# pola-rs/polars

Hardware: NVIDIA H100
Metric: group_by_agg_rows_per_sec (higher is better)
Workload: dtype int64/float64

## Files before the change

polars_b200/csrc/groupby_radix.cu:

```cuda
#include <algorithm>
#include <cstdlib>

#include "common.cuh"
#include "dev_utils.cuh"
#include "groupby.h"
#include "groupby_dev.cuh"

namespace plb {

constexpr int GBR_THREADS = 512;
constexpr int GBR_MAX_LOGB = 13;
constexpr int GBR_NCW = 31, GBR_NCT = GBR_NCW * 32;
constexpr unsigned GBR_NO_ROOM = 0xFFFFFFFFu;

struct GbRadixDev {
    uint64_t* recs;
    const unsigned long long* off;
    unsigned* cursor;
    unsigned* counts;
    int logB, roww;
    uint64_t* special;
    unsigned cap;
    int* status;
};

template <int KEY_ELEM> __device__ __forceinline__ void gbr_load_pair(const void* col, int64_t r0, int64_t n, uint64_t& a, uint64_t& b) {
    a = 0; b = 0;
    if (r0 + 1 < n) gb_load_pair<KEY_ELEM>(col, r0, a, b);
    else if (r0 < n) a = KEY_ELEM == 8 ? reinterpret_cast<const uint64_t*>(col)[r0] : reinterpret_cast<const uint32_t*>(col)[r0];
}
__device__ __forceinline__ void gbr_load_pair_rt(const void* col, int elem, int64_t r0, int64_t n, uint64_t& a, uint64_t& b) {
    if (elem == 8) gbr_load_pair<8>(col, r0, n, a, b); else gbr_load_pair<4>(col, r0, n, a, b);
}

template <int KEY_ELEM, int KEY_CANON>
__global__ void __launch_bounds__(512) k_gbr_hist(const void* __restrict__ keys, int64_t n, int logB, unsigned* __restrict__ counts) {
    extern __shared__ unsigned h_s[];
    const int B = 1 << logB;
    for (int i = threadIdx.x; i < B; i += blockDim.x) h_s[i] = 0;
    __syncthreads();
    const int64_t npairs = (n + 1) >> 1;
    for (int64_t p = (int64_t)blockIdx.x * blockDim.x + threadIdx.x; p < npairs; p += (int64_t)gridDim.x * blockDim.x) {
        uint64_t k0, k1;
        gbr_load_pair<KEY_ELEM>(keys, 2 * p, n, k0, k1);
        k0 = canon_key<KEY_CANON>(k0); k1 = canon_key<KEY_CANON>(k1);
        if (k0 != GB_EMPTY) atomicAdd(&h_s[(unsigned)(table_hash(k0) >> (64 - logB))], 1u);
        if (2 * p + 1 < n && k1 != GB_EMPTY) atomicAdd(&h_s[(unsigned)(table_hash(k1) >> (64 - logB))], 1u);
    }
    __syncthreads();
    for (int i = threadIdx.x; i < B; i += blockDim.x) if (h_s[i]) atomicAdd(&counts[i], h_s[i]);
}
__host__ __device__ __forceinline__ unsigned long long gbr_stream_records(unsigned long long rows, unsigned long long pad_units, unsigned pad_each, unsigned align) {
    rows += (rows < pad_units ? rows : pad_units) * pad_each;
    return (rows + align - 1) & ~(unsigned long long)(align - 1);
}
__global__ void __launch_bounds__(1024) k_gbr_offsets(const __grid_constant__ GbLayout L, const unsigned* __restrict__ counts, unsigned long long rows, int B, unsigned long long pad_units,
                                                      unsigned pad_each, unsigned align, unsigned long long* __restrict__ off, unsigned* __restrict__ cursor, uint64_t* __restrict__ special, int* __restrict__ status) {
// ... 17 lines not shown
            wsum[lane] = t - s;
        }
        __syncthreads();
        const unsigned long long incl = carry_s + wsum[warp] + x;
        if (i < B) off[i] = incl - c;
        __syncthreads();
        if (threadIdx.x == 1023) carry_s = incl;
        __syncthreads();
    }
    if (threadIdx.x == 0) off[B] = carry_s;
}

__device__ __forceinline__ void gbr_apply_special(const GbLayout& L, const GbBatch& Bt, uint64_t* sp, const uint64_t* raw) {
    atomicAdd(reinterpret_cast<unsigned long long*>(sp), 1ull);
    for (int c = 0; c < L.n_cols; c++)
        for (int k = L.col_kbegin[c]; k < L.col_kbegin[c + 1]; k++) {
            uint64_t* a = sp + 1 + L.wslot[k];
            const int dt = Bt.cols[c].dtype;
            switch (L.wop[k]) {
                case W_ADD_INT: atomicAdd(reinterpret_cast<unsigned long long*>(a), (unsigned long long)raw_to_int(dt, raw[c])); break;
                case W_ADD_F64: atomicAdd(reinterpret_cast<double*>(a), raw_to_f64(dt, raw[c])); break;
                case W_MIN_S64: atomicMin(reinterpret_cast<long long*>(a), (long long)raw_to_int(dt, raw[c])); break;
                case W_MAX_S64: atomicMax(reinterpret_cast<long long*>(a), (long long)raw_to_int(dt, raw[c])); break;
                case W_MIN_U64: atomicMin(reinterpret_cast<unsigned long long*>(a), (unsigned long long)raw[c]); break;
                case W_MAX_U64: atomicMax(reinterpret_cast<unsigned long long*>(a), (unsigned long long)raw[c]); break;
                case W_MIN_F64: { const double f = raw_to_f64(dt, raw[c]); if (f == f) atomicMin(reinterpret_cast<unsigned long long*>(a), (unsigned long long)f64_to_ordered(f)); break; }
                case W_MAX_F64: { const double f = raw_to_f64(dt, raw[c]); if (f == f) atomicMax(reinterpret_cast<unsigned long long*>(a), (unsigned long long)f64_to_ordered(f)); break; }
                default: break;
            }
        }
}

constexpr int GBR_RPT = 4;
template <int ROWW, int KEY_ELEM, int KEY_CANON, bool BULK>
__global__ void __launch_bounds__(GBR_THREADS) k_gbr_scatter(const __grid_constant__ GbLayout L, const __grid_constant__ GbBatch Bt, const __grid_constant__ GbRadixDev R) {
    constexpr int RPT = GBR_RPT, T = GBR_THREADS * RPT, THREADS = GBR_THREADS, NC = ROWW - 1;
    const int logB = R.logB, B = 1 << logB;
    extern __shared__ __align__(16) uint64_t gbr_smem[];
    uint64_t* stage = gbr_smem;
    unsigned* hist = reinterpret_cast<unsigned*>(stage + (size_t)(T + (BULK ? B : 0)) * ROWW);
    unsigned* start = hist + B;
    unsigned* gpos = start + B;
    uint16_t* sp = reinterpret_cast<uint16_t*>(gpos + B);
    __shared__ unsigned warp_tot[THREADS / 32];
    const int tid = threadIdx.x, lane = tid & 31, warp = tid >> 5;
    const int64_t n = Bt.n;
    const int64_t ntiles = (n + T - 1) / T;
    for (int64_t tile = blockIdx.x; tile < ntiles; tile += gridDim.x) {
        const int64_t base = tile * T;
        for (int p = tid; p < B; p += THREADS) hist[p] = 0;
        __syncthreads();
        uint64_t k[RPT]; unsigned pk[RPT];
#pragma unroll
        for (int j = 0; j < RPT / 2; j++) gbr_load_pair<KEY_ELEM>(Bt.keys, base + 2 * (int64_t)(j * THREADS + tid), n, k[2 * j], k[2 * j + 1]);
#pragma unroll
        for (int j = 0; j < RPT; j++) {
            const int64_t r = base + 2 * (int64_t)((j >> 1) * THREADS + tid) + (j & 1);
            pk[j] = 0xFFFFFFFFu;
            if (r < n) {
                k[j] = canon_key<KEY_CANON>(k[j]);
                if (k[j] == GB_EMPTY) pk[j] = 0xFFFFFFFEu;
                else { const unsigned b = (unsigned)(table_hash(k[j]) >> (64 - logB)); pk[j] = (b << 16) | atomicAdd(&hist[b], 1u); }
            }
        }
        __syncthreads();
        const int bins = (B + THREADS - 1) / THREADS;
        unsigned mine = 0;
        for (int q = 0; q < bins; q++) { const int p = tid * bins + q; if (p < B) { unsigned c = hist[p]; if (BULK) c = (c + 1u) & ~1u; mine += c; } }
        unsigned x = mine;
        for (int o = 1; o < 32; o <<= 1) { const unsigned y = __shfl_up_sync(0xffffffffu, x, o); if (lane >= o) x += y; }
        if (lane == 31) warp_tot[warp] = x;
        __syncthreads();
        if (warp == 0) {
            unsigned w = lane < THREADS / 32 ? warp_tot[lane] : 0, s = w;
            for (int o = 1; o < 32; o <<= 1) { const unsigned y = __shfl_up_sync(0xffffffffu, s, o); if (lane >= o) s += y; }
            if (lane < THREADS / 32) warp_tot[lane] = s - w;
        }
        __syncthreads();
        unsigned run = warp_tot[warp] + x - mine;
        for (int q = 0; q < bins; q++) {
            const int p = tid * bins + q;
            if (p < B) {
                const unsigned c = hist[p], cp = BULK ? ((c + 1u) & ~1u) : c;
                start[p] = run;
                unsigned g = cp ? atomicAdd(&R.cursor[p], cp) : 0u;
                if (g + cp > R.cap) { *R.status = 2; g = GBR_NO_ROOM; }
                gpos[p] = g;
                run += cp;
            }
        }
        if (BULK) bulk_wait_read0();
        __syncthreads();
        if (BULK) for (int p = tid; p < B; p += THREADS) { const unsigned c = hist[p]; if (c & 1u) { uint64_t* pad = stage + (size_t)(start[p] + c) * ROWW; pad[0] = GB_EMPTY;
#pragma unroll
                                                                                                      for (int w = 1; w < ROWW; w++) pad[w] = 0; } }
#pragma unroll
        for (int j = 0; j < RPT / 2; j++) {
            const int64_t r0 = base + 2 * (int64_t)(j * THREADS + tid);
            uint64_t v[NC > 0 ? NC : 1][2];
#pragma unroll
            for (int c = 0; c < NC; c++) gbr_load_pair_rt(Bt.cols[c].values, Bt.cols[c].elem, r0, n, v[c][0], v[c][1]);
#pragma unroll
            for (int e = 0; e < 2; e++) {
                const unsigned q = pk[2 * j + e];
                if (q == 0xFFFFFFFFu) continue;
                if (q == 0xFFFFFFFEu) {
                    uint64_t raw[NC > 0 ? NC : 1];
#pragma unroll
                    for (int c = 0; c < NC; c++) raw[c] = v[c][e];
                    gbr_apply_special(L, Bt, R.special, raw);
                    continue;
                }
                const unsigned bkt = q >> 16, pos = start[bkt] + (q & 0xFFFFu);
                uint64_t* rec = stage + (size_t)pos * ROWW;
                rec[0] = k[2 * j + e];
#pragma unroll
                for (int c = 0; c < NC; c++) rec[1 + c] = v[c][e];
                if (!BULK) sp[pos] = (uint16_t)bkt;
            }
        }
        if (BULK) fence_async_smem();
        __syncthreads();
        if (BULK) {
            for (int p = tid; p < B; p += THREADS) {
                const unsigned c = hist[p], cp = (c + 1u) & ~1u;
                if (cp && gpos[p] != GBR_NO_ROOM) bulk_s2g(R.recs + (R.off[p] + gpos[p]) * ROWW, stage + (size_t)start[p] * ROWW, cp * ROWW * 8);
            }
            bulk_commit();
        } else {
            const unsigned total = start[B - 1] + hist[B - 1];
            for (unsigned w = tid; w < total * ROWW; w += THREADS) {
                const unsigned row = w / ROWW, c = w - row * ROWW;
                const unsigned p = sp[row], g = gpos[p];
                if (g != GBR_NO_ROOM) R.recs[(R.off[p] + g + (row - start[p])) * ROWW + c] = stage[w];
            }
            __syncthreads();
        }
    }
    if (BULK) bulk_wait0();
}

constexpr int GBR_WC_THREADS = 256, GBR_WC_F = 4;
template <int ROWW> constexpr int gbr_wc_rpt() { return ROWW <= 3 ? 8 : 4; }
template <int ROWW, int KEY_ELEM, int RPT>
__device__ __forceinline__ void gbr_wc_load(const GbBatch& Bt, int64_t base, uint64_t (&k)[RPT], uint64_t (&v)[ROWW > 1 ? ROWW - 1 : 1][RPT]) {
#pragma unroll
    for (int j = 0; j < RPT / 2; j++) {
        const int64_t r0 = base + 2 * (int64_t)(j * GBR_WC_THREADS + threadIdx.x);
        gbr_load_pair<KEY_ELEM>(Bt.keys, r0, Bt.n, k[2 * j], k[2 * j + 1]);
#pragma unroll
        for (int c = 0; c < ROWW - 1; c++) gbr_load_pair_rt(Bt.cols[c].values, Bt.cols[c].elem, r0, Bt.n, v[c][2 * j], v[c][2 * j + 1]);
    }
}

template <int ROWW, int KEY_ELEM, int KEY_CANON>
__global__ void __launch_bounds__(GBR_WC_THREADS, 2) k_gbr_scatter_wc(const __grid_constant__ GbLayout L, const __grid_constant__ GbBatch Bt, const __grid_constant__ GbRadixDev R) {
    constexpr int THREADS = GBR_WC_THREADS, F = GBR_WC_F, RPT = gbr_wc_rpt<ROWW>(), T = THREADS * RPT, NC = ROWW - 1, NCX = NC > 0 ? NC : 1, CH = F * ROWW;
    constexpr unsigned NONE = 0xFFFFFFFFu;
    const int logB = R.logB, B = 1 << logB, tid = threadIdx.x;
    extern __shared__ __align__(16) uint64_t gbr_smem[];
    uint64_t* buf = gbr_smem;
    unsigned* fill = reinterpret_cast<unsigned*>(buf + (size_t)B * CH);
    const int64_t n = Bt.n, ntiles = (n + T - 1) / T;
    for (int p = tid; p < B; p += THREADS) fill[p] = 0;
    uint64_t k[RPT], v[NCX][RPT], kn[RPT], vn[NCX][RPT];
    if ((int64_t)blockIdx.x < ntiles) gbr_wc_load<ROWW, KEY_ELEM, RPT>(Bt, (int64_t)blockIdx.x * T, kn, vn);
    for (int64_t tile = blockIdx.x; tile < ntiles; tile += gridDim.x) {
#pragma unroll
        for (int e = 0; e < RPT; e++) { k[e] = kn[e];
#pragma unroll
                                        for (int c = 0; c < NC; c++) v[c][e] = vn[c][e]; }
        if (tile + gridDim.x < ntiles) gbr_wc_load<ROWW, KEY_ELEM, RPT>(Bt, (tile + gridDim.x) * T, kn, vn);
        const int64_t base = tile * T;
        unsigned pk[RPT];
#pragma unroll
        for (int e = 0; e < RPT; e++) {
            const int64_t r = base + 2 * (int64_t)((e >> 1) * THREADS + tid) + (e & 1);
            pk[e] = NONE;
            if (r < n) {
                k[e] = canon_key<KEY_CANON>(k[e]);
                if (k[e] == GB_EMPTY) {
                    uint64_t raw[NCX];
#pragma unroll
                    for (int c = 0; c < NC; c++) raw[c] = v[c][e];
                    gbr_apply_special(L, Bt, R.special, raw);
                } else pk[e] = (unsigned)(table_hash(k[e]) >> (64 - logB)) << 16;
            }
        }
        __syncthreads();
        unsigned last = 0;
#pragma unroll
        for (int e = 0; e < RPT; e++)
            if (pk[e] != NONE) { const unsigned s = atomicAdd(&fill[pk[e] >> 16], 1u); pk[e] |= s; last = max(last, s / F); }
        bulk_wait_read0();
        __syncthreads();
        for (unsigned r = 0;; r++) {
#pragma unroll
            for (int e = 0; e < RPT; e++) {
                const unsigned s = pk[e] & 0xFFFFu;
                if (pk[e] == NONE || s / F != r) continue;
                uint64_t* rec = buf + (size_t)(pk[e] >> 16) * CH + (s % F) * ROWW;
                rec[0] = k[e];
#pragma unroll
                for (int c = 0; c < NC; c++) rec[1 + c] = v[c][e];
            }
            fence_async_smem();
            const bool more = __syncthreads_or(last > r);
            const unsigned full = (r + 1) * F;
            for (int p0 = 0; p0 < B; p0 += 4 * THREADS) {
                unsigned g[4];
#pragma unroll
                for (int q = 0; q < 4; q++) {
                    const int p = p0 + q * THREADS + tid;
                    g[q] = NONE;
                    if (p < B) {
                        const unsigned f = fill[p];
                        if (f >= full) g[q] = atomicAdd(&R.cursor[p], (unsigned)F);
                        if (!more) fill[p] = f % F;
                    }
                }
#pragma unroll
                for (int q = 0; q < 4; q++) {
                    const int p = p0 + q * THREADS + tid;
                    if (g[q] == NONE) continue;
                    if (g[q] + F <= R.cap) bulk_s2g(R.recs + (R.off[p] + g[q]) * ROWW, buf + (size_t)p * CH, CH * 8);
                    else *R.status = 2;
                }
            }
            bulk_commit();
            if (!more) break;
            bulk_wait_read0();
            __syncthreads();
        }
    }
    __syncthreads();
    for (int p = tid; p < B; p += THREADS) {
        const unsigned f = fill[p];
        if (f == 0) continue;
        for (unsigned i = f; i < F; i++) buf[(size_t)p * CH + i * ROWW] = GB_EMPTY;
        fence_async_smem();
        const unsigned g = atomicAdd(&R.cursor[p], (unsigned)F);
        if (g + F <= R.cap) bulk_s2g(R.recs + (R.off[p] + g) * ROWW, buf + (size_t)p * CH, CH * 8);
        else *R.status = 2;
    }
    bulk_commit();
    bulk_wait0();
}

struct GbDenseDev { uint64_t* keys; uint32_t* first; uint32_t* len; uint64_t* words; int64_t Gb; unsigned long long* cursor; };

constexpr int GBR_NST = 2;
template <int ROWW>
__global__ void __launch_bounds__(1024) k_gbr_agg(const __grid_constant__ GbLayout L, const __grid_constant__ GbBatch Bt, const __grid_constant__ GbRadixDev R, const __grid_constant__ GbDenseDev D, unsigned S) {
    constexpr int NST = GBR_NST, CR = GBR_NCT, NC = ROWW - 1;
    extern __shared__ __align__(128) uint64_t gbr_smem2[];
    uint64_t* ring = gbr_smem2;
    uint64_t* tkey = ring + (size_t)NST * CR * ROWW;
    uint64_t* tacc = tkey + S;
    unsigned* tlen = reinterpret_cast<unsigned*>(tacc + (size_t)L.n_words * S);
    __shared__ uint64_t full[NST], empty[NST];
    __shared__ unsigned s_used, s_base;
    const int tid = threadIdx.x, warp = tid >> 5, lane = tid & 31, B = 1 << R.logB;
    if (*R.status == 2) return;
    if (tid == 0) { for (int s = 0; s < NST; s++) { mbar_init(&full[s], 1); mbar_init(&empty[s], GBR_NCW); } mbar_fence_init(); }
    __syncthreads();
    if (warp == GBR_NCW) {
        if (lane == 0) {
            unsigned q = 0;
            for (int p = blockIdx.x; p < B; p += gridDim.x) {
                const int64_t rows = (int64_t)R.cursor[p];
                const uint64_t* src = R.recs + R.off[p] * ROWW;
                const int nch = (int)((rows + CR - 1) / CR);
                for (int c = 0; c < nch; c++, q++) {
                    const int st = q % NST; const unsigned use = q / NST;
                    if (use > 0) while (!mbar_try_wait(&empty[st], (use - 1) & 1u)) {}
                    const int64_t crow = min((int64_t)CR, rows - (int64_t)c * CR);
                    const unsigned bytes = (unsigned)(((crow + 1) & ~(int64_t)1) * ROWW * 8);
                    mbar_expect_tx(&full[st], bytes);
                    bulk_g2s(ring + (size_t)st * CR * ROWW, src + (size_t)c * CR * ROWW, bytes, &full[st]);
                }
            }
        }
        return;
    }
    const unsigned max_used = S - (S >> 2);
    unsigned q = 0;
    for (int p = blockIdx.x; p < B; p += gridDim.x) {
        for (unsigned i = tid; i < S; i += GBR_NCT) { tkey[i] = GB_EMPTY; tlen[i] = 0; for (int w = 0; w < L.n_words; w++) tacc[(size_t)w * S + i] = L.init[w]; }
        if (tid == 0) s_used = 0;
        named_bar_sync(1, GBR_NCT);
        const int64_t rows = (int64_t)R.cursor[p];
        const int nch = (int)((rows + CR - 1) / CR);
        for (int c = 0; c < nch; c++, q++) {
            const int st = q % NST; const unsigned par = (q / NST) & 1u;
            while (!mbar_try_wait(&full[st], par)) {}
            const uint64_t* buf = ring + (size_t)st * CR * ROWW;
            const int crow = (int)min((int64_t)CR, rows - (int64_t)c * CR);
            uint64_t rec[ROWW];
            rec[0] = GB_EMPTY;
            if (tid < crow) {
#pragma unroll
                for (int w = 0; w < ROWW; w++) rec[w] = buf[tid * ROWW + w];
            }
            fence_async_smem();
            __syncwarp();
            if (lane == 0) mbar_arrive(&empty[st]);
            const uint64_t key = rec[0];
            if (key == GB_EMPTY) continue;
            unsigned slot = __umulhi((unsigned)((table_hash(key) << R.logB) >> 32), S);
            bool found = false;
            for (unsigned probes = 0; probes < 128u; probes++) {
                const uint64_t cur = *reinterpret_cast<volatile uint64_t*>(tkey + slot);
                if (cur == key) { found = true; break; }
                if (cur == GB_EMPTY) {
                    if (*reinterpret_cast<volatile unsigned*>(&s_used) >= max_used) break;
                    const unsigned long long old = atomicCAS(reinterpret_cast<unsigned long long*>(tkey + slot), (unsigned long long)GB_EMPTY, (unsigned long long)key);
                    if (old == GB_EMPTY) { atomicAdd(&s_used, 1u); found = true; break; }
                    if (old == key) { found = true; break; }
                }
                if (++slot == S) slot = 0;
            }
            if (!found) { *R.status = 1; continue; }
            if (L.need_len) atomicAdd(tlen + slot, 1u);
#pragma unroll
            for (int cix = 0; cix < NC; cix++) {
                const int dt = Bt.cols[cix].dtype;
                for (int kk = L.col_kbegin[cix]; kk < L.col_kbegin[cix + 1]; kk++) gb_apply_smem<false>(L.wop[kk], tacc + (size_t)L.wslot[kk] * S + slot, dt, rec[1 + cix], true);
            }
        }
        named_bar_sync(1, GBR_NCT);
        if (tid == 0) s_base = (unsigned)atomicAdd(D.cursor, (unsigned long long)s_used);
        named_bar_sync(1, GBR_NCT);
        const unsigned long long base = s_base;
        for (unsigned i0 = 0; i0 < S; i0 += GBR_NCT) {
            const unsigned i = i0 + tid;
            const bool used = i < S && tkey[i] != GB_EMPTY;
            unsigned at = 0;
            if (used) at = atomicSub(&s_used, 1u) - 1u;
            if (used) {
                const unsigned long long pos = base + at;
                if ((int64_t)pos >= D.Gb) *R.status = 1;
                else {
                    D.keys[pos] = tkey[i]; D.len[pos] = tlen[i]; D.first[pos] = 0xFFFFFFFFu;
                    for (int w = 0; w < L.n_words; w++) D.words[(int64_t)w * D.Gb + pos] = tacc[(size_t)w * S + i];
                }
            }
        }
        named_bar_sync(1, GBR_NCT);
    }
}

__global__ void k_gbr_append_special(const uint64_t* __restrict__ special, int n_words, GbDenseDev D, int* status) {
    if (threadIdx.x != 0 || blockIdx.x != 0 || special[0] == 0) return;
    const unsigned long long pos = atomicAdd(D.cursor, 1ull);
    if ((int64_t)pos >= D.Gb) { *status = 1; return; }
    D.keys[pos] = GB_EMPTY; D.len[pos] = (uint32_t)special[0]; D.first[pos] = 0xFFFFFFFFu;
    for (int w = 0; w < n_words; w++) D.words[(int64_t)w * D.Gb + pos] = special[1 + w];
}

static size_t gbr_wc_smem(int B, int roww) { return (size_t)B * (GBR_WC_F * roww * 8 + 4); }
static size_t gbr_scatter_smem(int B, int roww, bool bulk) {
    const size_t tile = (size_t)GBR_THREADS * GBR_RPT;
    return (tile + (bulk ? B : 0)) * roww * 8 + (size_t)3 * B * 4 + (bulk ? 0 : tile * 2);
}
template <int ROWW, int KEY_ELEM, int KEY_CANON>
static int scatter_wc_grid(int B) {
    auto kfn = k_gbr_scatter_wc<ROWW, KEY_ELEM, KEY_CANON>;
    const size_t smem = gbr_wc_smem(B, ROWW);
    PLB_CUDA(cudaFuncSetAttribute(kfn, cudaFuncAttributeMaxDynamicSharedMemorySize, (int)smem));
    int occ = 0;
    PLB_CUDA(cudaOccupancyMaxActiveBlocksPerMultiprocessor(&occ, kfn, GBR_WC_THREADS, smem));
    return ctx().sm_count * std::max(occ, 1);
}
template <int ROWW, int KEY_ELEM, int KEY_CANON>
static void launch_scatter(const GbLayout& L, const GbBatch& Bt, const GbRadixDev& R, bool bulk) {
    const size_t smem = gbr_scatter_smem(1 << R.logB, ROWW, bulk);
    auto kfn = bulk ? k_gbr_scatter<ROWW, KEY_ELEM, KEY_CANON, true> : k_gbr_scatter<ROWW, KEY_ELEM, KEY_CANON, false>;
    PLB_CUDA(cudaFuncSetAttribute(kfn, cudaFuncAttributeMaxDynamicSharedMemorySize, (int)smem));
    int occ = 0;
    PLB_CUDA(cudaOccupancyMaxActiveBlocksPerMultiprocessor(&occ, kfn, GBR_THREADS, smem));
    PLB_LAUNCH("k5r_scatter", kfn, ctx().sm_count * std::max(occ, 1), GBR_THREADS, smem, L, Bt, R);
}
template <int ROWW>
static void launch_agg(const GbLayout& L, const GbBatch& Bt, const GbRadixDev& R, const GbDenseDev& D, unsigned S) {
    auto kfn = k_gbr_agg<ROWW>;
    const size_t smem = (size_t)GBR_NST * GBR_NCT * ROWW * 8 + (size_t)S * (8 + 4 + 8 * L.n_words) + 16;
    PLB_CUDA(cudaFuncSetAttribute(kfn, cudaFuncAttributeMaxDynamicSharedMemorySize, (int)smem));
    int occ = 0;
    PLB_CUDA(cudaOccupancyMaxActiveBlocksPerMultiprocessor(&occ, kfn, 1024, smem));
    PLB_LAUNCH("k5r_aggregate", kfn, std::min(1 << R.logB, ctx().sm_count * std::max(occ, 1)), 1024, smem, L, Bt, R, D, S);
}

bool GroupByState::consume_radix(const DevCol& key, const std::vector<const DevCol*>& values, uint64_t planned_cap) {
    const int mode = knob_int("BL_K5_RADIX", 1);
    if (mode == 0 || L.need_first || key.validity != nullptr || hot.rows > 0 || key.len < (1 << 20)) return false;
    for (size_t i = 0; i < plans.size(); i++) {
        if (plans[i].kind == BL_AGG_LEN) continue;
        const DevCol* v = values[i];
        if (v == nullptr || v->len != key.len || v->dtype != plans[i].in_dtype || v->validity != nullptr) return false;
        if (dtype_size(v->dtype) != 4 && dtype_size(v->dtype) != 8) return false;
    }
    GbBatch Bt; GbLayout Lb;
    if (!bind_columns(key, values, 0, 0, 4, Bt, Lb)) return false;
    const int roww = 1 + Lb.n_cols;
    const int64_t n = key.len;
    const size_t entry = 8 + 4 + 8 * (size_t)L.n_words;
    const size_t ring2 = (size_t)GBR_NST * GBR_NCT * roww * 8;
    unsigned S = 0; int logB = 6;
    for (const size_t total_kb : {(size_t)110, (size_t)222}) {
        if (total_kb * 1024 < ring2 + 1024 + 512 * entry) continue;
        S = (unsigned)((total_kb * 1024 - ring2 - 1024) / entry) & ~31u;
        const double per_bucket = 0.55 * (double)S;
        logB = 6;
        while (logB < GBR_MAX_LOGB && (double)est_groups / (double)(1 << logB) > per_bucket) logB++;
        if ((double)est_groups / (double)(1 << logB) <= 0.7 * (double)S) break;
        S = 0;
    }
    if (S == 0) return false;
    if (mode == 1) {
        const double l2_budget = 0.55 * (double)ctx().l2_bytes;
        if ((double)planned_cap * L.stride * 8 <= 2.0 * l2_budget) return false;
    }
    const int B = 1 << logB;
    int smem_optin = 0;
    PLB_CUDA(cudaDeviceGetAttribute(&smem_optin, cudaDevAttrMaxSharedMemoryPerBlockOptin, ctx().device));
    const bool wc_fits = gbr_wc_smem(B, roww) <= (size_t)smem_optin;
    const int store = knob_int("BL_K5R_STORE", 0);
    bool bulk = logB <= 9, wc = !bulk && wc_fits;
    if (store == 1 && gbr_scatter_smem(B, roww, false) <= (size_t)smem_optin) bulk = wc = false;
    else if (store == 2 && wc_fits) { bulk = false; wc = true; }
    else if (store == 3 && gbr_scatter_smem(B, roww, true) <= (size_t)smem_optin) { bulk = true; wc = false; }
    const int64_t ntiles = (n + GBR_THREADS * GBR_RPT - 1) / (GBR_THREADS * GBR_RPT);
    auto with_scatter_form = [&](auto f) { with_key_form(key.dtype, [&](auto e, auto c) { with_at_least<1, 2, 3, 4, 5>(roww, [&](auto w) { f(e, c, w); }); }); };
    int wc_grid = 0;
    if (wc) with_scatter_form([&](auto e, auto c, auto w) { wc_grid = scatter_wc_grid<decltype(w)::value, decltype(e)::value, decltype(c)::value>(B); });
    const unsigned long long pad_units = wc ? (unsigned long long)wc_grid : (unsigned long long)ntiles;
    const unsigned pad_each = wc ? GBR_WC_F - 1 : bulk ? 1u : 0u, align = wc ? GBR_WC_F : 2u;
    const double mean = (double)n / B, margin = 5.0 * std::sqrt(est_f2 / B);
    unsigned long long bucket_rows = est_f2 > 0 && margin <= 0.5 * mean ? (unsigned long long)std::ceil(mean + margin) : 0;
    const int64_t exact_rows = n + std::min<int64_t>(n, (int64_t)B * (int64_t)pad_units) * pad_each + (int64_t)align * B + 16;
    int64_t rec_rows = bucket_rows ? (int64_t)B * (int64_t)gbr_stream_records(bucket_rows, pad_units, pad_each, align) + 16 : exact_rows;
    DevPtr recs, ctl;
    try {
        recs = dev_alloc((size_t)rec_rows * roww * 8);
        ctl = dev_alloc((size_t)B * 4 * 2 + (size_t)(B + 1) * 8 + (size_t)(1 + GB_MAX_WORDS) * 8 + 64);
    } catch (const Error&) { cudaGetLastError(); return false; }
    GbRadixDev R; memset(&R, 0, sizeof R);
    R.recs = as<uint64_t>(recs); R.logB = logB; R.roww = roww; R.status = as<int>(status);
    char* cp = reinterpret_cast<char*>(ctl->p);
    R.off = reinterpret_cast<unsigned long long*>(cp); cp += (size_t)(B + 1) * 8;
    R.special = reinterpret_cast<uint64_t*>(cp); cp += (size_t)(1 + GB_MAX_WORDS) * 8;
    R.counts = reinterpret_cast<unsigned*>(cp); cp += (size_t)B * 4;
    R.cursor = reinterpret_cast<unsigned*>(cp);
    const int64_t Gb = std::max<int64_t>(1024, std::min<int64_t>(n + 1, 3 * est_groups + (1 << 16)));
    dense.keys = dev_alloc((size_t)Gb * 8); dense.first = dev_alloc((size_t)Gb * 4); dense.len = dev_alloc((size_t)Gb * 4);
    dense.words = dev_alloc((size_t)Gb * 8 * std::max(L.n_words, 1)); dense.ctl = dev_alloc(16); dense.Gb = Gb;
    GbDenseDev D{as<uint64_t>(dense.keys), as<uint32_t>(dense.first), as<uint32_t>(dense.len), as<uint64_t>(dense.words), Gb, as<unsigned long long>(dense.ctl)};
    for (;;) {
        const unsigned long long cap = bucket_rows ? gbr_stream_records(bucket_rows, pad_units, pad_each, align) : 0;
        R.cap = cap ? (unsigned)cap : ~0u;
        if (!bucket_rows) {
            dev_memset(R.counts, 0, (size_t)B * 4);
            with_key_form(key.dtype, [&](auto e, auto c) {
                PLB_LAUNCH("k5r_histogram", (k_gbr_hist<decltype(e)::value, decltype(c)::value>), ctx().sm_count * 4, 512, (size_t)B * 4, key.v(), n, logB, R.counts);
            });
        }
        PLB_LAUNCH("k5r_setup", k_gbr_offsets, 1, 1024, 0, L, bucket_rows ? nullptr : R.counts, bucket_rows, B, pad_units, pad_each, align,
                   const_cast<unsigned long long*>(R.off), R.cursor, R.special, R.status);
        with_scatter_form([&](auto e, auto c, auto w) {
            constexpr int E = decltype(e)::value, C = decltype(c)::value, ROWW = decltype(w)::value;
            if (wc) PLB_LAUNCH("k5r_scatter", (k_gbr_scatter_wc<ROWW, E, C>), wc_grid, GBR_WC_THREADS, gbr_wc_smem(B, ROWW), Lb, Bt, R);
            else launch_scatter<ROWW, E, C>(Lb, Bt, R, bulk);
        });
        dev_memset(dense.ctl->p, 0, 8); dev_memset(static_cast<char*>(dense.ctl->p) + 8, 0xFF, 8);
        with_at_least<1, 2, 3, 4, 5>(roww, [&](auto w) { launch_agg<decltype(w)::value>(Lb, Bt, R, D, S); });
        PLB_LAUNCH("k5r_special", k_gbr_append_special, 1, 32, 0, R.special, L.n_words, D, as<int>(status));
        const int st = read_scalar(as<int>(status));
        if (getenv("BL_K5_DEBUG"))
            fprintf(stderr, "[k5r] rows=%lld est_groups=%lld buckets=%d slots=%u bulk=%d store=%s sizing=%s cap=%llu status=%d\n", (long long)n, (long long)est_groups, B, S, (int)bulk,
                    bulk ? "runs" : wc ? "wc" : "coalesced", bucket_rows ? "sample" : "exact", cap, st);
        if (st == 2 && bucket_rows) {
            bucket_rows = 0;
            if (exact_rows > rec_rows) {
                recs.reset();
                try { recs = dev_alloc((size_t)exact_rows * roww * 8); } catch (const Error&) { cudaGetLastError(); dense = GbDense{}; dev_memset(status->p, 0, 4); return false; }
                R.recs = as<uint64_t>(recs); rec_rows = exact_rows;
            }
            continue;
        }
        if (st != 0) { dense = GbDense{}; dev_memset(status->p, 0, 4); return false; }
        dense.ready = true;
        rows_seen = n;
        return true;
    }
}

}
```

Measured before the change: 28.51 billion.

## Pack radix scatter records into narrow 32-bit fields using sampled value ranges

```diff
diff --git a/polars_b200/csrc/groupby_radix.cu b/polars_b200/csrc/groupby_radix.cu
--- a/polars_b200/csrc/groupby_radix.cu
+++ b/polars_b200/csrc/groupby_radix.cu
@@ -1,4 +1,5 @@
 #include <algorithm>
+#include <climits>
 #include <cstdlib>
 
 #include "common.cuh"
@@ -12,6 +13,26 @@
 constexpr int GBR_MAX_LOGB = 13;
 constexpr int GBR_NCW = 31, GBR_NCT = GBR_NCW * 32;
 constexpr unsigned GBR_NO_ROOM = 0xFFFFFFFFu;
+constexpr int GBR_ST_TABLE = 1, GBR_ST_STREAM = 2, GBR_ST_LAYOUT = 4;
+
+enum { GBR_F8 = 0, GBR_Z4 = 1, GBR_S4 = 2 };
+constexpr int GBR_PACK_COLS = 2;
+constexpr uint32_t GBR_PAD32 = 0xFFFFFFFFu;
+struct GbRecLayout {
+    uint64_t kbase, kmask;
+    int32_t kslot;
+    int32_t vkind[GBR_PACK_COLS], vslot[GBR_PACK_COLS];
+};
+__host__ __device__ constexpr int gbr_slot(int lay, int nc, int f) {
+    int s = 0;
+    for (int c = 0; c < nc; c++)
+        if (((lay >> 2 * c) & 3) == GBR_F8) { if (f == 1 + c) return s; s += 2; }
+    if (f == 0) return s;
+    s++;
+    for (int c = 0; c < nc; c++)
+        if (((lay >> 2 * c) & 3) != GBR_F8) { if (f == 1 + c) return s; s++; }
+    return s;
+}
 
 struct GbRadixDev {
     uint64_t* recs;
@@ -22,7 +43,49 @@
     uint64_t* special;
     unsigned cap;
     int* status;
+    GbRecLayout P;
 };
+
+template <int RECW> __device__ __forceinline__ void gbr_put(uint64_t (&w)[RECW], int slot, uint64_t x) {
+    x <<= (slot & 1) * 32;
+#pragma unroll
+    for (int i = 0; i < RECW; i++) w[i] |= x & (0ull - (uint64_t)((slot >> 1) == i));
+}
+template <int NC, int RECW, class Val>
+__device__ __forceinline__ bool gbr_pack(const GbRecLayout& P, uint64_t (&w)[RECW], uint64_t key, Val val) {
+#pragma unroll
+    for (int i = 0; i < RECW; i++) w[i] = 0;
+    const uint64_t kd = (key - P.kbase) & P.kmask;
+    bool ok = kd < GBR_PAD32;
+    gbr_put(w, P.kslot, kd);
+#pragma unroll
+    for (int c = 0; c < NC; c++) {
+        const uint64_t x = val(c);
+        const bool f8 = P.vkind[c] == GBR_F8;
+        ok &= f8 || (P.vkind[c] == GBR_S4 ? (uint64_t)(long long)(int)(uint32_t)x == x : (x >> 32) == 0);
+        gbr_put(w, P.vslot[c], f8 ? x : x & 0xFFFFFFFFull);
+    }
+    return ok;
+}
+template <int LAY, int NC, int F, int RECW> __device__ __forceinline__ uint64_t gbr_unpack(const uint64_t (&w)[RECW]) {
+    constexpr int S = gbr_slot(LAY, NC, F), KIND = F == 0 ? GBR_Z4 : (LAY >> 2 * (F - 1)) & 3;
+    const uint64_t x = w[S / 2];
+    if constexpr (KIND == GBR_F8) return x;
+    const uint32_t h = (S & 1) ? (uint32_t)(x >> 32) : (uint32_t)x;
+    return KIND == GBR_S4 ? (uint64_t)(long long)(int)h : (uint64_t)h;
+}
+template <int RECW> __device__ __forceinline__ void gbr_ld_rec(const uint64_t* p, uint64_t (&w)[RECW]) {
+#pragma unroll
+    for (int i = 0; i + 1 < RECW; i += 2) { const ulonglong2 t = reinterpret_cast<const ulonglong2*>(p)[i / 2]; w[i] = t.x; w[i + 1] = t.y; }
+    if (RECW % 2) w[RECW - 1] = p[RECW - 1];
+}
+template <int RECW> __device__ __forceinline__ void gbr_st_rec(uint64_t* p, const uint64_t (&w)[RECW]) {
+#pragma unroll
+    for (int i = 0; i + 1 < RECW; i += 2) reinterpret_cast<ulonglong2*>(p)[i / 2] = make_ulonglong2(w[i], w[i + 1]);
+    if (RECW % 2) p[RECW - 1] = w[RECW - 1];
+}
+__device__ __forceinline__ void gbr_pad(const GbRecLayout& P, uint64_t* rec) { reinterpret_cast<uint32_t*>(rec)[P.kslot] = GBR_PAD32; }
+
 
 template <int KEY_ELEM> __device__ __forceinline__ void gbr_load_pair(const void* col, int64_t r0, int64_t n, uint64_t& a, uint64_t& b) {
     a = 0; b = 0;
@@ -106,13 +169,14 @@
 }
 
 constexpr int GBR_RPT = 4;
-template <int ROWW, int KEY_ELEM, int KEY_CANON, bool BULK>
+template <int ROWW, int RECW, int KEY_ELEM, int KEY_CANON, bool BULK>
 __global__ void __launch_bounds__(GBR_THREADS) k_gbr_scatter(const __grid_constant__ GbLayout L, const __grid_constant__ GbBatch Bt, const __grid_constant__ GbRadixDev R) {
     constexpr int RPT = GBR_RPT, T = GBR_THREADS * RPT, THREADS = GBR_THREADS, NC = ROWW - 1;
+    constexpr bool PACK = RECW < ROWW;
     const int logB = R.logB, B = 1 << logB;
     extern __shared__ __align__(16) uint64_t gbr_smem[];
     uint64_t* stage = gbr_smem;
-    unsigned* hist = reinterpret_cast<unsigned*>(stage + (size_t)(T + (BULK ? B : 0)) * ROWW);
+    unsigned* hist = reinterpret_cast<unsigned*>(stage + (size_t)(T + (BULK ? B : 0)) * RECW);
     unsigned* start = hist + B;
     unsigned* gpos = start + B;
     uint16_t* sp = reinterpret_cast<uint16_t*>(gpos + B);
@@ -158,16 +222,18 @@
                 const unsigned c = hist[p], cp = BULK ? ((c + 1u) & ~1u) : c;
                 start[p] = run;
                 unsigned g = cp ? atomicAdd(&R.cursor[p], cp) : 0u;
-                if (g + cp > R.cap) { *R.status = 2; g = GBR_NO_ROOM; }
+                if (g + cp > R.cap) { atomicOr(R.status, GBR_ST_STREAM); g = GBR_NO_ROOM; }
                 gpos[p] = g;
                 run += cp;
             }
         }
         if (BULK) bulk_wait_read0();
         __syncthreads();
-        if (BULK) for (int p = tid; p < B; p += THREADS) { const unsigned c = hist[p]; if (c & 1u) { uint64_t* pad = stage + (size_t)(start[p] + c) * ROWW; pad[0] = GB_EMPTY;
-#pragma unroll
-                                                                                                      for (int w = 1; w < ROWW; w++) pad[w] = 0; } }
+        if (BULK) for (int p = tid; p < B; p += THREADS) { const unsigned c = hist[p]; if (c & 1u) { uint64_t* pad = stage + (size_t)(start[p] + c) * RECW;
+                                                                                                      if constexpr (PACK) gbr_pad(R.P, pad);
+                                                                                                      else { pad[0] = GB_EMPTY;
+#pragma unroll
+                                                                                                             for (int w = 1; w < ROWW; w++) pad[w] = 0; } } }
 #pragma unroll
         for (int j = 0; j < RPT / 2; j++) {
             const int64_t r0 = base + 2 * (int64_t)(j * THREADS + tid);
@@ -186,10 +252,16 @@
                     continue;
                 }
                 const unsigned bkt = q >> 16, pos = start[bkt] + (q & 0xFFFFu);
-                uint64_t* rec = stage + (size_t)pos * ROWW;
-                rec[0] = k[2 * j + e];
-#pragma unroll
-                for (int c = 0; c < NC; c++) rec[1 + c] = v[c][e];
+                uint64_t* rec = stage + (size_t)pos * RECW;
+                if constexpr (PACK) {
+                    uint64_t w[RECW];
+                    if (gbr_pack<NC>(R.P, w, k[2 * j + e], [&](int c) { return v[c][e]; })) gbr_st_rec<RECW>(rec, w);
+                    else atomicOr(R.status, GBR_ST_LAYOUT);
+                } else {
+                    rec[0] = k[2 * j + e];
+#pragma unroll
+                    for (int c = 0; c < NC; c++) rec[1 + c] = v[c][e];
+                }
                 if (!BULK) sp[pos] = (uint16_t)bkt;
             }
         }
@@ -198,15 +270,15 @@
         if (BULK) {
             for (int p = tid; p < B; p += THREADS) {
                 const unsigned c = hist[p], cp = (c + 1u) & ~1u;
-                if (cp && gpos[p] != GBR_NO_ROOM) bulk_s2g(R.recs + (R.off[p] + gpos[p]) * ROWW, stage + (size_t)start[p] * ROWW, cp * ROWW * 8);
+                if (cp && gpos[p] != GBR_NO_ROOM) bulk_s2g(R.recs + (R.off[p] + gpos[p]) * RECW, stage + (size_t)start[p] * RECW, cp * RECW * 8);
             }
             bulk_commit();
         } else {
             const unsigned total = start[B - 1] + hist[B - 1];
-            for (unsigned w = tid; w < total * ROWW; w += THREADS) {
-                const unsigned row = w / ROWW, c = w - row * ROWW;
+            for (unsigned w = tid; w < total * RECW; w += THREADS) {
+                const unsigned row = w / RECW, c = w - row * RECW;
                 const unsigned p = sp[row], g = gpos[p];
-                if (g != GBR_NO_ROOM) R.recs[(R.off[p] + g + (row - start[p])) * ROWW + c] = stage[w];
+                if (g != GBR_NO_ROOM) R.recs[(R.off[p] + g + (row - start[p])) * RECW + c] = stage[w];
             }
             __syncthreads();
         }
@@ -227,9 +299,10 @@
     }
 }
 
-template <int ROWW, int KEY_ELEM, int KEY_CANON>
+template <int ROWW, int RECW, int KEY_ELEM, int KEY_CANON>
 __global__ void __launch_bounds__(GBR_WC_THREADS, 2) k_gbr_scatter_wc(const __grid_constant__ GbLayout L, const __grid_constant__ GbBatch Bt, const __grid_constant__ GbRadixDev R) {
-    constexpr int THREADS = GBR_WC_THREADS, F = GBR_WC_F, RPT = gbr_wc_rpt<ROWW>(), T = THREADS * RPT, NC = ROWW - 1, NCX = NC > 0 ? NC : 1, CH = F * ROWW;
+    constexpr int THREADS = GBR_WC_THREADS, F = GBR_WC_F, RPT = gbr_wc_rpt<ROWW>(), T = THREADS * RPT, NC = ROWW - 1, NCX = NC > 0 ? NC : 1, CH = F * RECW;
+    constexpr bool PACK = RECW < ROWW;
     constexpr unsigned NONE = 0xFFFFFFFFu;
     const int logB = R.logB, B = 1 << logB, tid = threadIdx.x;
     extern __shared__ __align__(16) uint64_t gbr_smem[];
@@ -244,9 +317,10 @@
         for (int e = 0; e < RPT; e++) { k[e] = kn[e];
 #pragma unroll
                                         for (int c = 0; c < NC; c++) v[c][e] = vn[c][e]; }
-        if (tile + gridDim.x < ntiles) gbr_wc_load<ROWW, KEY_ELEM, RPT>(Bt, (tile + gridDim.x) * T, kn, vn);
+        if (!PACK && tile + gridDim.x < ntiles) gbr_wc_load<ROWW, KEY_ELEM, RPT>(Bt, (tile + gridDim.x) * T, kn, vn);
         const int64_t base = tile * T;
         unsigned pk[RPT];
+        uint64_t pw[PACK ? RECW : 1][RPT];
 #pragma unroll
         for (int e = 0; e < RPT; e++) {
             const int64_t r = base + 2 * (int64_t)((e >> 1) * THREADS + tid) + (e & 1);
@@ -258,9 +332,18 @@
 #pragma unroll
                     for (int c = 0; c < NC; c++) raw[c] = v[c][e];
                     gbr_apply_special(L, Bt, R.special, raw);
-                } else pk[e] = (unsigned)(table_hash(k[e]) >> (64 - logB)) << 16;
-            }
-        }
+                } else {
+                    pk[e] = (unsigned)(table_hash(k[e]) >> (64 - logB)) << 16;
+                    if constexpr (PACK) {
+                        uint64_t w[RECW];
+                        if (!gbr_pack<NC>(R.P, w, k[e], [&](int c) { return v[c][e]; })) { atomicOr(R.status, GBR_ST_LAYOUT); pk[e] = NONE; }
+#pragma unroll
+                        for (int i = 0; i < RECW; i++) pw[i][e] = w[i];
+                    }
+                }
+            }
+        }
+        if (PACK && tile + gridDim.x < ntiles) gbr_wc_load<ROWW, KEY_ELEM, RPT>(Bt, (tile + gridDim.x) * T, kn, vn);
         __syncthreads();
         unsigned last = 0;
 #pragma unroll
@@ -273,10 +356,17 @@
             for (int e = 0; e < RPT; e++) {
                 const unsigned s = pk[e] & 0xFFFFu;
                 if (pk[e] == NONE || s / F != r) continue;
-                uint64_t* rec = buf + (size_t)(pk[e] >> 16) * CH + (s % F) * ROWW;
-                rec[0] = k[e];
-#pragma unroll
-                for (int c = 0; c < NC; c++) rec[1 + c] = v[c][e];
+                uint64_t* rec = buf + (size_t)(pk[e] >> 16) * CH + (s % F) * RECW;
+                if constexpr (PACK) {
+                    uint64_t w[RECW];
+#pragma unroll
+                    for (int i = 0; i < RECW; i++) w[i] = pw[i][e];
+                    gbr_st_rec<RECW>(rec, w);
+                } else {
+                    rec[0] = k[e];
+#pragma unroll
+                    for (int c = 0; c < NC; c++) rec[1 + c] = v[c][e];
+                }
             }
             fence_async_smem();
             const bool more = __syncthreads_or(last > r);
@@ -297,8 +387,8 @@
                 for (int q = 0; q < 4; q++) {
                     const int p = p0 + q * THREADS + tid;
                     if (g[q] == NONE) continue;
-                    if (g[q] + F <= R.cap) bulk_s2g(R.recs + (R.off[p] + g[q]) * ROWW, buf + (size_t)p * CH, CH * 8);
-                    else *R.status = 2;
+                    if (g[q] + F <= R.cap) bulk_s2g(R.recs + (R.off[p] + g[q]) * RECW, buf + (size_t)p * CH, CH * 8);
+                    else atomicOr(R.status, GBR_ST_STREAM);
                 }
             }
             bulk_commit();
@@ -311,11 +401,14 @@
     for (int p = tid; p < B; p += THREADS) {
         const unsigned f = fill[p];
         if (f == 0) continue;
-        for (unsigned i = f; i < F; i++) buf[(size_t)p * CH + i * ROWW] = GB_EMPTY;
+        for (unsigned i = f; i < F; i++) {
+            if constexpr (PACK) gbr_pad(R.P, buf + (size_t)p * CH + i * RECW);
+            else buf[(size_t)p * CH + i * ROWW] = GB_EMPTY;
+        }
         fence_async_smem();
         const unsigned g = atomicAdd(&R.cursor[p], (unsigned)F);
-        if (g + F <= R.cap) bulk_s2g(R.recs + (R.off[p] + g) * ROWW, buf + (size_t)p * CH, CH * 8);
-        else *R.status = 2;
+        if (g + F <= R.cap) bulk_s2g(R.recs + (R.off[p] + g) * RECW, buf + (size_t)p * CH, CH * 8);
+        else atomicOr(R.status, GBR_ST_STREAM);
     }
     bulk_commit();
     bulk_wait0();
@@ -324,18 +417,19 @@
 struct GbDenseDev { uint64_t* keys; uint32_t* first; uint32_t* len; uint64_t* words; int64_t Gb; unsigned long long* cursor; };
 
 constexpr int GBR_NST = 2;
-template <int ROWW>
+template <int ROWW, int RECW, int LAY>
 __global__ void __launch_bounds__(1024) k_gbr_agg(const __grid_constant__ GbLayout L, const __grid_constant__ GbBatch Bt, const __grid_constant__ GbRadixDev R, const __grid_constant__ GbDenseDev D, unsigned S) {
     constexpr int NST = GBR_NST, CR = GBR_NCT, NC = ROWW - 1;
+    constexpr bool PACK = RECW < ROWW;
     extern __shared__ __align__(128) uint64_t gbr_smem2[];
     uint64_t* ring = gbr_smem2;
-    uint64_t* tkey = ring + (size_t)NST * CR * ROWW;
+    uint64_t* tkey = ring + (size_t)NST * CR * RECW;
     uint64_t* tacc = tkey + S;
     unsigned* tlen = reinterpret_cast<unsigned*>(tacc + (size_t)L.n_words * S);
     __shared__ uint64_t full[NST], empty[NST];
     __shared__ unsigned s_used, s_base;
     const int tid = threadIdx.x, warp = tid >> 5, lane = tid & 31, B = 1 << R.logB;
-    if (*R.status == 2) return;
+    if (*R.status & (GBR_ST_STREAM | GBR_ST_LAYOUT)) return;
     if (tid == 0) { for (int s = 0; s < NST; s++) { mbar_init(&full[s], 1); mbar_init(&empty[s], GBR_NCW); } mbar_fence_init(); }
     __syncthreads();
     if (warp == GBR_NCW) {
@@ -343,15 +437,15 @@
             unsigned q = 0;
             for (int p = blockIdx.x; p < B; p += gridDim.x) {
                 const int64_t rows = (int64_t)R.cursor[p];
-                const uint64_t* src = R.recs + R.off[p] * ROWW;
+                const uint64_t* src = R.recs + R.off[p] * RECW;
                 const int nch = (int)((rows + CR - 1) / CR);
                 for (int c = 0; c < nch; c++, q++) {
                     const int st = q % NST; const unsigned use = q / NST;
                     if (use > 0) while (!mbar_try_wait(&empty[st], (use - 1) & 1u)) {}
                     const int64_t crow = min((int64_t)CR, rows - (int64_t)c * CR);
-                    const unsigned bytes = (unsigned)(((crow + 1) & ~(int64_t)1) * ROWW * 8);
+                    const unsigned bytes = (unsigned)(((crow + 1) & ~(int64_t)1) * RECW * 8);
                     mbar_expect_tx(&full[st], bytes);
-                    bulk_g2s(ring + (size_t)st * CR * ROWW, src + (size_t)c * CR * ROWW, bytes, &full[st]);
+                    bulk_g2s(ring + (size_t)st * CR * RECW, src + (size_t)c * CR * RECW, bytes, &full[st]);
                 }
             }
         }
@@ -368,18 +462,28 @@
         for (int c = 0; c < nch; c++, q++) {
             const int st = q % NST; const unsigned par = (q / NST) & 1u;
             while (!mbar_try_wait(&full[st], par)) {}
-            const uint64_t* buf = ring + (size_t)st * CR * ROWW;
+            const uint64_t* buf = ring + (size_t)st * CR * RECW;
             const int crow = (int)min((int64_t)CR, rows - (int64_t)c * CR);
             uint64_t rec[ROWW];
             rec[0] = GB_EMPTY;
             if (tid < crow) {
-#pragma unroll
-                for (int w = 0; w < ROWW; w++) rec[w] = buf[tid * ROWW + w];
+                if constexpr (PACK) {
+                    uint64_t w[RECW];
+                    gbr_ld_rec<RECW>(buf + tid * RECW, w);
+                    rec[0] = gbr_unpack<LAY, NC, 0>(w);
+                    if constexpr (NC >= 1) rec[1] = gbr_unpack<LAY, NC, 1>(w);
+                    if constexpr (NC >= 2) rec[2] = gbr_unpack<LAY, NC, 2>(w);
+                } else {
+#pragma unroll
+                    for (int w = 0; w < ROWW; w++) rec[w] = buf[tid * ROWW + w];
+                }
             }
             fence_async_smem();
             __syncwarp();
             if (lane == 0) mbar_arrive(&empty[st]);
-            const uint64_t key = rec[0];
+            uint64_t key = rec[0];
+            if constexpr (PACK)
+                if (tid < crow) key = key == GBR_PAD32 ? GB_EMPTY : (R.P.kbase + key) & R.P.kmask;
             if (key == GB_EMPTY) continue;
             unsigned slot = __umulhi((unsigned)((table_hash(key) << R.logB) >> 32), S);
             bool found = false;
@@ -424,6 +528,38 @@
     }
 }
 
+constexpr int GB_RADIX_MAX_COLS = 4;
+template <int KEY_ELEM, int KEY_CANON>
+__global__ void __launch_bounds__(1024) k_gbr_range(const __grid_constant__ GbBatch Bt, int nc, int64_t m, long long* __restrict__ out) {
+    constexpr int NF = 1 + GB_RADIX_MAX_COLS;
+    __shared__ long long lo_s[NF], hi_s[NF];
+    if (threadIdx.x < NF) { lo_s[threadIdx.x] = LLONG_MAX; hi_s[threadIdx.x] = LLONG_MIN; }
+    __syncthreads();
+    long long lo[NF], hi[NF];
+#pragma unroll
+    for (int f = 0; f < NF; f++) { lo[f] = LLONG_MAX; hi[f] = LLONG_MIN; }
+    for (int64_t i = (int64_t)blockIdx.x * blockDim.x + threadIdx.x; i < m; i += (int64_t)gridDim.x * blockDim.x) {
+        const int64_t row = (int64_t)(((unsigned __int128)i * (unsigned __int128)Bt.n) / (unsigned __int128)m);
+        const uint64_t k = canon_key<KEY_CANON>(KEY_ELEM == 8 ? reinterpret_cast<const uint64_t*>(Bt.keys)[row] : reinterpret_cast<const uint32_t*>(Bt.keys)[row]);
+        if (KEY_ELEM == 4 || k != GB_EMPTY) {
+            const long long x = KEY_ELEM == 8 ? (long long)k : (long long)(int)(uint32_t)k;
+            lo[0] = min(lo[0], x); hi[0] = max(hi[0], x);
+        }
+#pragma unroll
+        for (int c = 0; c < GB_RADIX_MAX_COLS; c++) {
+            if (c < nc) {
+                const GbColDev& col = Bt.cols[c];
+                const long long x = col.elem == 8 ? reinterpret_cast<const long long*>(col.values)[row] : (long long)reinterpret_cast<const uint32_t*>(col.values)[row];
+                lo[1 + c] = min(lo[1 + c], x); hi[1 + c] = max(hi[1 + c], x);
+            }
+        }
+    }
+#pragma unroll
+    for (int f = 0; f < NF; f++) { atomicMin(&lo_s[f], lo[f]); atomicMax(&hi_s[f], hi[f]); }
+    __syncthreads();
+    if (threadIdx.x < NF) { out[(size_t)blockIdx.x * 2 * NF + threadIdx.x] = lo_s[threadIdx.x]; out[(size_t)blockIdx.x * 2 * NF + NF + threadIdx.x] = hi_s[threadIdx.x]; }
+}
+
 __global__ void k_gbr_append_special(const uint64_t* __restrict__ special, int n_words, GbDenseDev D, int* status) {
     if (threadIdx.x != 0 || blockIdx.x != 0 || special[0] == 0) return;
     const unsigned long long pos = atomicAdd(D.cursor, 1ull);
@@ -437,32 +573,97 @@
     const size_t tile = (size_t)GBR_THREADS * GBR_RPT;
     return (tile + (bulk ? B : 0)) * roww * 8 + (size_t)3 * B * 4 + (bulk ? 0 : tile * 2);
 }
-template <int ROWW, int KEY_ELEM, int KEY_CANON>
+template <class F> static void with_rec_form(int roww, int recw, F&& f) {
+    if (recw == roww) with_at_least<1, 2, 3, 4, 5>(roww, [&](auto w) { f(w, w); });
+    else if (roww == 2 && recw == 1) f(IntC<2>{}, IntC<1>{});
+    else if (roww == 3 && recw == 2) f(IntC<3>{}, IntC<2>{});
+    else throw Error(BL_ERR_INVALID, "K5r: no kernel for this record width");
+}
+template <class F> static void with_agg_form(int roww, int recw, int lay, F&& f) {
+    if (recw == roww) { with_at_least<1, 2, 3, 4, 5>(roww, [&](auto w) { f(w, w, IntC<0>{}); }); return; }
+    auto one = [&](auto l) { if (lay == decltype(l)::value) { f(IntC<2>{}, IntC<1>{}, l); return true; } return false; };
+    auto two = [&](auto l) { if (lay == decltype(l)::value) { f(IntC<3>{}, IntC<2>{}, l); return true; } return false; };
+    constexpr int Z = GBR_Z4, SX = GBR_S4, F8 = GBR_F8;
+    const bool done = roww == 2 && recw == 1 ? one(IntC<Z>{}) || one(IntC<SX>{})
+                    : roww == 3 && recw == 2 ? two(IntC<Z | F8 << 2>{}) || two(IntC<SX | F8 << 2>{}) || two(IntC<F8 | Z << 2>{}) || two(IntC<F8 | SX << 2>{}) ||
+                                               two(IntC<Z | Z << 2>{}) || two(IntC<Z | SX << 2>{}) || two(IntC<SX | Z << 2>{}) || two(IntC<SX | SX << 2>{})
+                    : false;
+    if (!done) throw Error(BL_ERR_INVALID, "K5r: no kernel for this record layout");
+}
+template <int ROWW, int RECW, int KEY_ELEM, int KEY_CANON>
 static int scatter_wc_grid(int B) {
-    auto kfn = k_gbr_scatter_wc<ROWW, KEY_ELEM, KEY_CANON>;
-    const size_t smem = gbr_wc_smem(B, ROWW);
+    auto kfn = k_gbr_scatter_wc<ROWW, RECW, KEY_ELEM, KEY_CANON>;
+    const size_t smem = gbr_wc_smem(B, RECW);
     PLB_CUDA(cudaFuncSetAttribute(kfn, cudaFuncAttributeMaxDynamicSharedMemorySize, (int)smem));
     int occ = 0;
     PLB_CUDA(cudaOccupancyMaxActiveBlocksPerMultiprocessor(&occ, kfn, GBR_WC_THREADS, smem));
     return ctx().sm_count * std::max(occ, 1);
 }
-template <int ROWW, int KEY_ELEM, int KEY_CANON>
+template <int ROWW, int RECW, int KEY_ELEM, int KEY_CANON>
 static void launch_scatter(const GbLayout& L, const GbBatch& Bt, const GbRadixDev& R, bool bulk) {
-    const size_t smem = gbr_scatter_smem(1 << R.logB, ROWW, bulk);
-    auto kfn = bulk ? k_gbr_scatter<ROWW, KEY_ELEM, KEY_CANON, true> : k_gbr_scatter<ROWW, KEY_ELEM, KEY_CANON, false>;
+    const size_t smem = gbr_scatter_smem(1 << R.logB, RECW, bulk);
+    auto kfn = bulk ? k_gbr_scatter<ROWW, RECW, KEY_ELEM, KEY_CANON, true> : k_gbr_scatter<ROWW, RECW, KEY_ELEM, KEY_CANON, false>;
     PLB_CUDA(cudaFuncSetAttribute(kfn, cudaFuncAttributeMaxDynamicSharedMemorySize, (int)smem));
     int occ = 0;
     PLB_CUDA(cudaOccupancyMaxActiveBlocksPerMultiprocessor(&occ, kfn, GBR_THREADS, smem));
     PLB_LAUNCH("k5r_scatter", kfn, ctx().sm_count * std::max(occ, 1), GBR_THREADS, smem, L, Bt, R);
 }
-template <int ROWW>
+template <int ROWW, int RECW, int LAY>
 static void launch_agg(const GbLayout& L, const GbBatch& Bt, const GbRadixDev& R, const GbDenseDev& D, unsigned S) {
-    auto kfn = k_gbr_agg<ROWW>;
-    const size_t smem = (size_t)GBR_NST * GBR_NCT * ROWW * 8 + (size_t)S * (8 + 4 + 8 * L.n_words) + 16;
+    auto kfn = k_gbr_agg<ROWW, RECW, LAY>;
+    const size_t smem = (size_t)GBR_NST * GBR_NCT * RECW * 8 + (size_t)S * (8 + 4 + 8 * L.n_words) + 16;
     PLB_CUDA(cudaFuncSetAttribute(kfn, cudaFuncAttributeMaxDynamicSharedMemorySize, (int)smem));
     int occ = 0;
     PLB_CUDA(cudaOccupancyMaxActiveBlocksPerMultiprocessor(&occ, kfn, 1024, smem));
     PLB_LAUNCH("k5r_aggregate", kfn, std::min(1 << R.logB, ctx().sm_count * std::max(occ, 1)), 1024, smem, L, Bt, R, D, S);
+}
+
+static int gbr_rec_layout(const GbBatch& Bt, int nc, GbRecLayout& P, int& lay) {
+    const int roww = 1 + nc;
+    if (nc > GBR_PACK_COLS) return roww;
+    int best = 4;
+    for (int c = 0; c < nc; c++) best += Bt.cols[c].dtype == BL_FLOAT64 ? 8 : 4;
+    if ((best + 7) / 8 >= roww) return roww;
+    constexpr int NF = 1 + GB_RADIX_MAX_COLS;
+    const int64_t m = std::min<int64_t>(Bt.n, 65536);
+    const int grid = (int)std::min<int64_t>(64, (m + 1023) / 1024);
+    DevPtr buf = dev_alloc((size_t)grid * 2 * NF * 8);
+    with_key_form(Bt.key_dtype, [&](auto e, auto c) {
+        PLB_LAUNCH("k5r_sample", (k_gbr_range<decltype(e)::value, decltype(c)::value>), grid, 1024, 0, Bt, nc, m, as<long long>(buf));
+    });
+    std::vector<long long> h((size_t)grid * 2 * NF);
+    PLB_CUDA(cudaMemcpyAsync(h.data(), buf->p, h.size() * 8, cudaMemcpyDeviceToHost, ctx().stream));
+    PLB_CUDA(cudaStreamSynchronize(ctx().stream));
+    long long lo[NF], hi[NF];
+    for (int f = 0; f < NF; f++) {
+        lo[f] = LLONG_MAX; hi[f] = LLONG_MIN;
+        for (int b = 0; b < grid; b++) { lo[f] = std::min(lo[f], h[(size_t)b * 2 * NF + f]); hi[f] = std::max(hi[f], h[(size_t)b * 2 * NF + NF + f]); }
+    }
+    memset(&P, 0, sizeof P);
+    const uint64_t half = 1ull << 31;
+    if (dtype_size(Bt.key_dtype) == 4) {
+        const long long centre = lo[0] <= hi[0] ? lo[0] + (hi[0] - lo[0]) / 2 : 0;
+        P.kmask = 0xFFFFFFFFull; P.kbase = ((uint64_t)centre - half) & P.kmask;
+    } else if (lo[0] <= hi[0] && (uint64_t)hi[0] - (uint64_t)lo[0] < half) {
+        P.kmask = ~0ull; P.kbase = (uint64_t)lo[0] + ((uint64_t)hi[0] - (uint64_t)lo[0]) / 2 - half;
+    } else return roww;
+    int n8 = 0, n4 = 1;
+    lay = 0;
+    for (int c = 0; c < nc; c++) {
+        const long long a = lo[1 + c], b = hi[1 + c];
+        switch (Bt.cols[c].dtype) {
+            case BL_INT64: P.vkind[c] = a >= -(long long)(1 << 30) && b < (1 << 30) ? GBR_S4 : GBR_F8; break;
+            case BL_UINT64: P.vkind[c] = a >= 0 && b < (long long)half ? GBR_Z4 : GBR_F8; break;
+            default: P.vkind[c] = dtype_size(Bt.cols[c].dtype) == 4 ? GBR_Z4 : GBR_F8; break;
+        }
+        if (P.vkind[c] == GBR_F8) n8++; else n4++;
+        lay |= P.vkind[c] << 2 * c;
+    }
+    const int recw = (8 * n8 + 4 * n4 + 7) / 8;
+    if (recw >= roww) return roww;
+    P.kslot = gbr_slot(lay, nc, 0);
+    for (int c = 0; c < nc; c++) P.vslot[c] = gbr_slot(lay, nc, 1 + c);
+    return recw;
 }
 
 bool GroupByState::consume_radix(const DevCol& key, const std::vector<const DevCol*>& values, uint64_t planned_cap) {
@@ -505,22 +706,26 @@
     else if (store == 2 && wc_fits) { bulk = false; wc = true; }
     else if (store == 3 && gbr_scatter_smem(B, roww, true) <= (size_t)smem_optin) { bulk = true; wc = false; }
     const int64_t ntiles = (n + GBR_THREADS * GBR_RPT - 1) / (GBR_THREADS * GBR_RPT);
-    auto with_scatter_form = [&](auto f) { with_key_form(key.dtype, [&](auto e, auto c) { with_at_least<1, 2, 3, 4, 5>(roww, [&](auto w) { f(e, c, w); }); }); };
+    GbRecLayout P;
+    int lay = 0, recw = gbr_rec_layout(Bt, Lb.n_cols, P, lay);
+    auto with_scatter_form = [&](int rw, auto f) { with_key_form(key.dtype, [&](auto e, auto c) { with_rec_form(roww, rw, [&](auto w, auto r) { f(e, c, w, r); }); }); };
     int wc_grid = 0;
-    if (wc) with_scatter_form([&](auto e, auto c, auto w) { wc_grid = scatter_wc_grid<decltype(w)::value, decltype(e)::value, decltype(c)::value>(B); });
+    if (wc) with_scatter_form(roww, [&](auto e, auto c, auto w, auto r) { wc_grid = scatter_wc_grid<decltype(w)::value, decltype(r)::value, decltype(e)::value, decltype(c)::value>(B); });
+    if (wc && recw < roww) with_scatter_form(recw, [&](auto e, auto c, auto w, auto r) { scatter_wc_grid<decltype(w)::value, decltype(r)::value, decltype(e)::value, decltype(c)::value>(B); });
     const unsigned long long pad_units = wc ? (unsigned long long)wc_grid : (unsigned long long)ntiles;
     const unsigned pad_each = wc ? GBR_WC_F - 1 : bulk ? 1u : 0u, align = wc ? GBR_WC_F : 2u;
     const double mean = (double)n / B, margin = 5.0 * std::sqrt(est_f2 / B);
     unsigned long long bucket_rows = est_f2 > 0 && margin <= 0.5 * mean ? (unsigned long long)std::ceil(mean + margin) : 0;
     const int64_t exact_rows = n + std::min<int64_t>(n, (int64_t)B * (int64_t)pad_units) * pad_each + (int64_t)align * B + 16;
-    int64_t rec_rows = bucket_rows ? (int64_t)B * (int64_t)gbr_stream_records(bucket_rows, pad_units, pad_each, align) + 16 : exact_rows;
+    const int64_t rec_rows = bucket_rows ? (int64_t)B * (int64_t)gbr_stream_records(bucket_rows, pad_units, pad_each, align) + 16 : exact_rows;
     DevPtr recs, ctl;
+    size_t rec_bytes = (size_t)rec_rows * recw * 8;
     try {
-        recs = dev_alloc((size_t)rec_rows * roww * 8);
+        recs = dev_alloc(rec_bytes);
         ctl = dev_alloc((size_t)B * 4 * 2 + (size_t)(B + 1) * 8 + (size_t)(1 + GB_MAX_WORDS) * 8 + 64);
     } catch (const Error&) { cudaGetLastError(); return false; }
     GbRadixDev R; memset(&R, 0, sizeof R);
-    R.recs = as<uint64_t>(recs); R.logB = logB; R.roww = roww; R.status = as<int>(status);
+    R.recs = as<uint64_t>(recs); R.logB = logB; R.roww = roww; R.status = as<int>(status); R.P = P;
     char* cp = reinterpret_cast<char*>(ctl->p);
     R.off = reinterpret_cast<unsigned long long*>(cp); cp += (size_t)(B + 1) * 8;
     R.special = reinterpret_cast<uint64_t*>(cp); cp += (size_t)(1 + GB_MAX_WORDS) * 8;
@@ -541,24 +746,27 @@
         }
         PLB_LAUNCH("k5r_setup", k_gbr_offsets, 1, 1024, 0, L, bucket_rows ? nullptr : R.counts, bucket_rows, B, pad_units, pad_each, align,
                    const_cast<unsigned long long*>(R.off), R.cursor, R.special, R.status);
-        with_scatter_form([&](auto e, auto c, auto w) {
-            constexpr int E = decltype(e)::value, C = decltype(c)::value, ROWW = decltype(w)::value;
-            if (wc) PLB_LAUNCH("k5r_scatter", (k_gbr_scatter_wc<ROWW, E, C>), wc_grid, GBR_WC_THREADS, gbr_wc_smem(B, ROWW), Lb, Bt, R);
-            else launch_scatter<ROWW, E, C>(Lb, Bt, R, bulk);
+        with_scatter_form(recw, [&](auto e, auto c, auto w, auto r) {
+            constexpr int E = decltype(e)::value, C = decltype(c)::value, ROWW = decltype(w)::value, RECW = decltype(r)::value;
+            if (wc) PLB_LAUNCH("k5r_scatter", (k_gbr_scatter_wc<ROWW, RECW, E, C>), wc_grid, GBR_WC_THREADS, gbr_wc_smem(B, RECW), Lb, Bt, R);
+            else launch_scatter<ROWW, RECW, E, C>(Lb, Bt, R, bulk);
         });
         dev_memset(dense.ctl->p, 0, 8); dev_memset(static_cast<char*>(dense.ctl->p) + 8, 0xFF, 8);
-        with_at_least<1, 2, 3, 4, 5>(roww, [&](auto w) { launch_agg<decltype(w)::value>(Lb, Bt, R, D, S); });
+        with_agg_form(roww, recw, lay, [&](auto w, auto r, auto l) { launch_agg<decltype(w)::value, decltype(r)::value, decltype(l)::value>(Lb, Bt, R, D, S); });
         PLB_LAUNCH("k5r_special", k_gbr_append_special, 1, 32, 0, R.special, L.n_words, D, as<int>(status));
         const int st = read_scalar(as<int>(status));
         if (getenv("BL_K5_DEBUG"))
-            fprintf(stderr, "[k5r] rows=%lld est_groups=%lld buckets=%d slots=%u bulk=%d store=%s sizing=%s cap=%llu status=%d\n", (long long)n, (long long)est_groups, B, S, (int)bulk,
-                    bulk ? "runs" : wc ? "wc" : "coalesced", bucket_rows ? "sample" : "exact", cap, st);
-        if (st == 2 && bucket_rows) {
-            bucket_rows = 0;
-            if (exact_rows > rec_rows) {
+            fprintf(stderr, "[k5r] rows=%lld est_groups=%lld buckets=%d slots=%u bulk=%d store=%s sizing=%s cap=%llu rec=%d status=%d\n", (long long)n, (long long)est_groups, B, S, (int)bulk,
+                    bulk ? "runs" : wc ? "wc" : "coalesced", bucket_rows ? "sample" : "exact", cap, recw * 8, st);
+        const int redo = ((st & GBR_ST_STREAM) && bucket_rows ? GBR_ST_STREAM : 0) | ((st & GBR_ST_LAYOUT) && recw < roww ? GBR_ST_LAYOUT : 0);
+        if (redo && redo == st) {
+            if (st & GBR_ST_STREAM) bucket_rows = 0;
+            if (st & GBR_ST_LAYOUT) recw = roww;
+            const size_t need = (size_t)(bucket_rows ? rec_rows : exact_rows) * recw * 8;
+            if (need > rec_bytes) {
                 recs.reset();
-                try { recs = dev_alloc((size_t)exact_rows * roww * 8); } catch (const Error&) { cudaGetLastError(); dense = GbDense{}; dev_memset(status->p, 0, 4); return false; }
-                R.recs = as<uint64_t>(recs); rec_rows = exact_rows;
+                try { recs = dev_alloc(need); } catch (const Error&) { cudaGetLastError(); dense = GbDense{}; dev_memset(status->p, 0, 4); return false; }
+                R.recs = as<uint64_t>(recs); rec_bytes = need;
             }
             continue;
         }
```

Measured after the change: 29.80 billion (median of 6 runs). 1.05x the previous value.
